# WujiangXu/AMID

Measured on AMD Instinct MI355X. Metric: train samples/sec, higher is better.
Workload: dtype f32; 1 GPU; cloth_sport_train75-shaped SASRec train step (BASELINE.json configs[1]); batch_per_gpu=256, global_batch=256, seq_len=50, emb_dim=128, hid_dim=32, neg=1, table_rows=894820, unique_rows_last_step=1921, input=HBM-resident batch pool, dropout=on (p=0.5), optimizer=Adam (dense-equivalent lazy rows), graph=True, steps_per_graph=1, parallelism=dp1

## Files before the change

amid_amd/csrc/sasrec_strip_px.hip:

```cpp
#include "common.h"
#include "rng.h"
#include "strip_gemm.h"
#include "strip_chain.h"
#include "seq_fwd.h"
#include "seq_bwd.h"
#include "seqn_parts.h"
#include "sort_phases.h"
#include "scorer_sum.h"
#include "strip_px.h"

namespace amid {

constexpr int PXB_WPS = 4, PXB_NS = 2, PXB_NW = PXB_WPS * PXB_NS, PXB_THREADS = 64 * PXB_NW;
constexpr int PXB_STAT_STRIP = 2 * 64 + 2 * 16, PXB_STAT = PXB_WPS * PXB_STAT_STRIP;
template <int D> constexpr size_t pxb_lds_floats(int chains = 1) {
    return (size_t)3 * (D * D / 2) + (size_t)PXB_WPS * XpStrip<D>::FLOATS + PXB_STAT + (size_t)chains * PXB_WPS * 2 * D;
}

struct PxbRow { unsigned off_own, phys; int local; bool ok; };
template <int D>
__device__ __forceinline__ PxbRow pxb_row(const StripGeom& sg, const StripTile& t, int si, int c0) {
    PxbRow r;
    int v = t.v0 + si * 16 + (lane_id() & 15);
    r.ok = v < t.nv;
    if (!r.ok) v = t.v0;
    if (sg.live != nullptr) {
        const int s = v / sg.T;
        r.local = sg.live[t.s0 + s] * sg.T + (v - s * sg.T);
    } else {
        r.local = v;
    }
    r.phys = (unsigned)t.g * (unsigned)sg.M + (unsigned)r.local;
    r.off_own = r.ok ? r.phys * (unsigned)(D * 4) + 16u * (unsigned)(lane_id() >> 4) + (unsigned)c0 * 64u : STRIP_OOB;
    return r;
}

template <class Add>
__device__ __forceinline__ void pxb_row_chain(float* __restrict__ stat, int si, int part, float& a, float& b, const Add& add) {
    typedef __attribute__((address_space(3))) float lf;
    float* ls = stat + si * PXB_STAT_STRIP;
    float* rs = ls + 2 * 64;
    const int lane = lane_id(), m = lane & 15;
    a = 0.f; b = 0.f;
    if (part == 0) { add(a, b); lds_st1(ls + lane, a); lds_st1(ls + 64 + lane, b); }
    lds_barrier();
    if (part != 0) {
        a = *(lf*)(ls + lane); b = *(lf*)(ls + 64 + lane);
        add(a, b);
        a = row_sum4(a); b = row_sum4(b);
        if (lane < 16) { lds_st1(rs + m, a); lds_st1(rs + 16 + m, b); }
    }
    lds_barrier();
    if (part == 0) { a = *(lf*)(rs + m); b = *(lf*)(rs + 16 + m); }
}

template <int D, int NCT>
__device__ __forceinline__ void pxb_ln_partials(float* __restrict__ scratch, int si, int c0, const PartRegs<NCT>& dgam, const PartRegs<NCT>& dbet) {
    const int lane = lane_id();
    float* mine = scratch + si * 2 * D;
#pragma unroll
    for (int c = 0; c < NCT; ++c) {
        f32x4 a, b;
#pragma unroll
        for (int r = 0; r < 4; ++r) { a[r] = col_sum16(dgam.v[c][r]); b[r] = col_sum16(dbet.v[c][r]); }
        if ((lane & 15) == 0) {
            lds_st4(mine + (c0 + c) * 16 + 4 * (lane >> 4), a);
            lds_st4(mine + D + (c0 + c) * 16 + 4 * (lane >> 4), b);
        }
    }
}
template <int D>
__device__ __forceinline__ void pxb_ln_partials_out(const float* __restrict__ scratch, float* __restrict__ part) {
    for (int e = threadIdx.x; e < 2 * D; e += PXB_THREADS)
        part[e] = (scratch[e] + scratch[2 * D + e]) + (scratch[4 * D + e] + scratch[6 * D + e]);
}

template <int D, int NCT>
__device__ __forceinline__ void pxb_ln_bwd(PartRegs<NCT>& DR, const PartRegs<NCT>& dbet, const PartRegs<NCT>& X, const PartRegs<NCT>& gam, bool have_stat,
                                           float mean, float& rstd, float eps, float* __restrict__ stat, int si, int part, PartRegs<NCT>& dgam,
                                           const f32x4 (*addend)[NCT] = nullptr, PartRegs<NCT>* uout = nullptr) {
    if (!have_stat) {
        float tot, qt, dummy;
        pxb_row_chain(stat, si, part, tot, dummy, [&](float& s, float&) {
#pragma unroll
            for (int c = 0; c < NCT; ++c) s += (X.v[c][0] + X.v[c][1]) + (X.v[c][2] + X.v[c][3]);
        });
        mean = tot * (1.0f / D);
        pxb_row_chain(stat, si, part, qt, dummy, [&](float& q, float&) {
#pragma unroll
            for (int c = 0; c < NCT; ++c)
#pragma unroll
                for (int r = 0; r < 4; ++r) { const float d = X.v[c][r] - mean; q = fmaf(d, d, q); }
        });
        rstd = 1.0f / sqrtf(qt * (1.0f / D) + eps);
    }
    float t1, t2;
    pxb_row_chain(stat, si, part, t1, t2, [&](float& s1, float& s2) {
#pragma unroll
        for (int c = 0; c < NCT; ++c) {
#pragma unroll
            for (int r = 0; r < 4; ++r) {
                const float dy = dbet.v[c][r];
                const float xh = (X.v[c][r] - mean) * rstd;
                float gy = gam.v[c][r] * dy;
                asm volatile("" : "+v"(gy));
                s1 += gy;
                s2 = fmaf(gy, xh, s2);
                float dg = dy * xh;
                asm volatile("" : "+v"(dg));
                dgam.v[c][r] = dg;
                DR.v[c][r] = gy;
            }
        }
    });
    const float c1 = t1 * (1.0f / D), c2 = t2 * (1.0f / D);
    {
#pragma clang fp contract(off)
#pragma unroll
        for (int c = 0; c < NCT; ++c)
#pragma unroll
            for (int r = 0; r < 4; ++r) {
                const float xh = (X.v[c][r] - mean) * rstd;
                const float u = __builtin_fmaf(-xh, c2, DR.v[c][r] - c1);
                if (uout != nullptr) uout->v[c][r] = u;
                DR.v[c][r] = addend != nullptr ? __builtin_fmaf(rstd, u, (*addend)[c][r]) : rstd * u;
            }
    }
}

template <int NCT>
__device__ __forceinline__ void xp_write_scaled(float* __restrict__ xps, int c0, const PartRegs<NCT>& u, float k) {
#pragma clang fp contract(off)
    const int lane = lane_id();
    auto split = [&](float ua, float ub) {
        WgSplit2 s;
        s.hi = wg_pack2(k * ua, k * ub);
        const float a1 = __builtin_fmaf(k, ua, -__uint_as_float(s.hi << 16)), b1 = __builtin_fmaf(k, ub, -__uint_as_float(s.hi & 0xffff0000u));
        s.mid = wg_pack2(a1, b1);
        const float a2 = a1 - __uint_as_float(s.mid << 16), b2 = b1 - __uint_as_float(s.mid & 0xffff0000u);
        s.lo = wg_pack2(a2, b2);
        return s;
    };
#pragma unroll
    for (int e = 0; e < NCT / 2; ++e) {
        const int st = c0 / 2 + e;
        const WgSplit2 p0 = split(u.v[2 * e][0], u.v[2 * e][1]), p1 = split(u.v[2 * e][2], u.v[2 * e][3]);
        const WgSplit2 p2 = split(u.v[2 * e + 1][0], u.v[2 * e + 1][1]), p3 = split(u.v[2 * e + 1][2], u.v[2 * e + 1][3]);
        lds_st4(xps + ((st * 3 + 0) * 64 + lane) * 4, __builtin_bit_cast(f32x4, amid_v4u{p0.hi, p1.hi, p2.hi, p3.hi}));
        lds_st4(xps + ((st * 3 + 1) * 64 + lane) * 4, __builtin_bit_cast(f32x4, amid_v4u{p0.mid, p1.mid, p2.mid, p3.mid}));
        lds_st4(xps + ((st * 3 + 2) * 64 + lane) * 4, __builtin_bit_cast(f32x4, amid_v4u{p0.lo, p1.lo, p2.lo, p3.lo}));
    }
}

template <int D, int NW> struct PxbRing : SeqRing3<D, NW> {
    using Base = SeqRing3<D, NW>;
    __device__ __forceinline__ explicit PxbRing(float* lds) : Base(lds) {}
    __device__ __forceinline__ void next() {
        w_ring_wait();
        __syncthreads();
        if (!this->hi_ready) this->plane(this->hslot(), this->cur);
    }
    __device__ __forceinline__ void mid_sync() {
        w_ring_wait();
        __syncthreads();
        this->plane(this->mslot(), this->nxt + (size_t)D * D);
        this->plane(this->lslot(), this->nxt + (size_t)2 * D * D);
        this->cur = this->nxt; this->hi_ready = false;
    }
};

template <int D, int NCT, class Ring>
__device__ __forceinline__ void pxb_mma_xp(f32x4 (&acc)[NCT], const float* __restrict__ xps, Ring& ring, int c0) {
    constexpr int KS = D / 32, NSTEP = KS * NCT, CT_BYTES = 16 * (D / 2) * 4, PLANE_BYTES = Ring::SLAB * 4;
    constexpr int PD1 = FRAG_AHEAD_2, PD2 = FRAG_AHEAD_1;
    static_assert(PD1 < NSTEP && PD2 < NSTEP && 2 * PD1 + 2 < 16, "read-ahead against the step count and the lgkmcnt field");
    const int lane = lane_id();
    const int i = lane & 15, g = lane >> 4;
    auto mma = [&](const f32x4& wf, const f32x4& a16, const f32x4& c) {
        return __builtin_amdgcn_mfma_f32_16x16x32_bf16(__builtin_bit_cast(seqn_bf16x8, wf), __builtin_bit_cast(seqn_bf16x8, a16), c, 0, 0, 0);
    };
    unsigned fo[KS];
#pragma unroll
    for (int s = 0; s < KS; ++s) fo[s] = (unsigned)((((c0 * 16 + i) * (D / 2)) + 4 * ((4 * s + g) ^ i)) * 4);
    const unsigned xa = lds_offset(xps) + (unsigned)lane * 16u;
    const unsigned mbase = lds_offset(ring.mslot());
    static_assert(CT_BYTES * (NCT - 1) + PLANE_BYTES < 65536, "the lo plane is reached through the offset field");
    const unsigned hbase = mbase + 2u * PLANE_BYTES;
    {
        f32x4 wm[PD1 + 1], wl[PD1 + 1], ah[KS], am[KS];
        static_for<KS>([&](auto S) {
            constexpr int s = decltype(S)::value;
            lds_frag_issue<(s * 3 + 0) * 1024>(ah[s], xa);
            lds_frag_issue<(s * 3 + 1) * 1024>(am[s], xa);
        });
        auto issue = [&](auto U) {
            constexpr int u = decltype(U)::value, c = u / KS, s = u % KS, k = u % (PD1 + 1);
            lds_frag_issue<c * CT_BYTES>(wm[k], mbase + fo[s]);
            lds_frag_issue<c * CT_BYTES + PLANE_BYTES>(wl[k], mbase + fo[s]);
        };
        static_for<PD1>(issue);
        static_for<NSTEP>([&](auto T) {
            constexpr int t = decltype(T)::value, c = t / KS, s = t % KS, k = t % (PD1 + 1);
            if constexpr (t + PD1 < NSTEP) issue(std::integral_constant<int, t + PD1>{});
            constexpr int last = t + PD1 < NSTEP ? t + PD1 : NSTEP - 1;
            asm volatile("s_waitcnt lgkmcnt(%4)" : "+v"(wm[k]), "+v"(wl[k]), "+v"(ah[s]), "+v"(am[s]) : "n"(2 * (last - t)));
            acc[c] = mma(wm[k], am[s], acc[c]); acc[c] = mma(wl[k], ah[s], acc[c]); acc[c] = mma(wm[k], ah[s], acc[c]);
        });
    }
    ring.mid_sync();
    {
        f32x4 wf[PD2 + 1], ah[KS], am[KS], al[KS];
        static_for<KS>([&](auto S) {
            constexpr int s = decltype(S)::value;
            lds_frag_issue<(s * 3 + 0) * 1024>(ah[s], xa);
            lds_frag_issue<(s * 3 + 1) * 1024>(am[s], xa);
            lds_frag_issue<(s * 3 + 2) * 1024>(al[s], xa);
        });
        auto issue = [&](auto U) {
            constexpr int u = decltype(U)::value, c = u / KS, s = u % KS;
            lds_frag_issue<c * CT_BYTES>(wf[u % (PD2 + 1)], hbase + fo[s]);
        };
        static_for<PD2>(issue);
        static_for<NSTEP>([&](auto T) {
            constexpr int t = decltype(T)::value, c = t / KS, s = t % KS, k = t % (PD2 + 1);
            if constexpr (t + PD2 < NSTEP) issue(std::integral_constant<int, t + PD2>{});
            constexpr int last = t + PD2 < NSTEP ? t + PD2 : NSTEP - 1;
            asm volatile("s_waitcnt lgkmcnt(%4)" : "+v"(wf[k]), "+v"(ah[s]), "+v"(am[s]), "+v"(al[s]) : "n"(last - t));
            acc[c] = mma(wf[k], al[s], acc[c]); acc[c] = mma(wf[k], am[s], acc[c]); acc[c] = mma(wf[k], ah[s], acc[c]);
        });
    }
}

template <int D, int NCT, bool ZERO = true, class Ring, class Stores>
__device__ __forceinline__ void pxb_product(f32x4 (&acc)[NCT], const float* __restrict__ xps, Ring& ring, const unsigned short* __restrict__ wn16, int c0,
                                            const Stores& stores) {
    if constexpr (ZERO) {
#pragma unroll
        for (int c = 0; c < NCT; ++c) acc[c] = f32x4{0.f, 0.f, 0.f, 0.f};
    }
    ring.begin(wn16);
#pragma unroll
    for (int ct = 0; ct < NCT; ++ct) { stores(ct, 1); stores(ct, 3); }
    pxb_mma_xp<D, NCT, Ring>(acc, xps, ring, c0);
}

template <int D, int NCT>
__device__ __forceinline__ void pxb_tm_load(unsigned (&bits)[NCT], const unsigned char* __restrict__ tmq, const StripGeom& sg, const PxbRow& row, int c0) {
    const GBuf gtm(tmq, sg.tm_bytes);
    const unsigned tbase = row.ok ? row.phys * (unsigned)(D / 4) + (unsigned)c0 * 4u : STRIP_OOB;
    const int sh = 8 * (lane_id() >> 4);
#pragma unroll
    for (int c = 0; c < NCT; ++c) bits[c] = (unsigned)__builtin_amdgcn_raw_buffer_load_b32(gtm.r, (int)(tbase + 4 * c), 0, 0) >> sh;
}
template <int NCT>
__device__ __forceinline__ void pxb_tm_apply(PartRegs<NCT>& x, const unsigned (&bits)[NCT]) {
#pragma unroll
    for (int c = 0; c < NCT; ++c) {
        x.v[c][0] = (bits[c] & 1u) ? 0.f : x.v[c][0];
        x.v[c][1] = (bits[c] & 2u) ? 0.f : x.v[c][1];
        x.v[c][2] = (bits[c] & 4u) ? 0.f : x.v[c][2];
        x.v[c][3] = (bits[c] & 8u) ? 0.f : x.v[c][3];
    }
}

template <int NCT> struct PxbFfnPre { PartRegs<NCT> Hs, gam; unsigned tm[NCT]; float mean, rstd; };
template <int D, int NCT>
__device__ __forceinline__ void pxb_ffn_prefetch(PxbFfnPre<NCT>& p, const StripFfnBwdArgs& a, const float* __restrict__ ln_stat, const StripGeom& sg,
                                                 const PxbRow& row, int g, int c0) {
    part_load<NCT>(p.Hs, GBuf(a.h, sg.act_bytes), row.off_own);
    if (a.tmq != nullptr) pxb_tm_load<D, NCT>(p.tm, a.tmq, sg, row, c0);
    part_cols<NCT>(p.gam, a.ln_w[g], c0);
    p.mean = 0.f; p.rstd = 0.f;
    if (ln_stat != nullptr && row.ok) { p.mean = ln_stat[(long long)row.phys * 4 + 2]; p.rstd = ln_stat[(long long)row.phys * 4 + 3]; }
}

template <int D, int NCT, class Ring>
__device__ __forceinline__ void pxb_ffn_bwd_chain(const StripFfnBwdArgs& a, const float* __restrict__ ln_stat, const StripGeom& sg, Ring& ring,
                                                  const PxbRow& row, int g, int si, int part, int c0, PartRegs<NCT>& DZ, PxbFfnPre<NCT>& pre,
                                                  float* __restrict__ xps, float* __restrict__ stat, float* __restrict__ lnsc,
                                                  const unsigned short* __restrict__ wnext) {
    const GBuf gp2(a.dpre2, sg.act_bytes), gp1(a.dpre1, sg.act_bytes), gdr(a.dr, sg.act_bytes), gdo(a.d_o, sg.act_bytes);
    PartRegs<NCT> P, Rs;
    PartRegs<NCT>& Hs = pre.Hs;
    PartRegs<NCT>& gam = pre.gam;
    float mean = pre.mean, rstd = pre.rstd;
    if (a.tmq != nullptr) pxb_tm_apply<NCT>(DZ, pre.tm);
    P = DZ;
    if (a.train) {
        const uint4 rr2 = rng_call(a.st->seed, (unsigned long long)row.local * D >> 7, site_id(g, a.layer, SITE_FFN2), (unsigned)a.st->step);
        part_dropout<NCT>(P, rr2, c0, a.spec, a.scale, (row.local * D) & 127);
    }
    xp_write<NCT>(xps, c0, P);
    f32x4 acc[NCT];
    {
        ring.next();
        part_load<NCT>(Rs, GBuf(a.r, sg.act_bytes), row.off_own);
        pxb_product<D, NCT>(acc, xps, ring, (const unsigned short*)a.w1T[g], c0, [&](int ct, int j) { part_spread<NCT>(gp2, row.off_own, P, ct, j, 1); });
#pragma unroll
        for (int c = 0; c < NCT; ++c)
#pragma unroll
            for (int r = 0; r < 4; ++r) P.v[c][r] = Hs.v[c][r] > 0.f ? acc[c][r] * a.scale : 0.f;
    }
    lds_barrier();
    xp_write<NCT>(xps, c0, P);
    PartRegs<NCT> DR, U, dgam, dbet;
    {
        ring.next();
        pxb_product<D, NCT>(acc, xps, ring, (const unsigned short*)a.woT[g], c0, [&](int ct, int j) { part_spread<NCT>(gp1, row.off_own, P, ct, j, 1); });
#pragma unroll
        for (int c = 0; c < NCT; ++c) dbet.v[c] = acc[c] + DZ.v[c];
        pxb_ln_bwd<D, NCT>(DR, dbet, Rs, gam, ln_stat != nullptr, mean, rstd, a.ln_eps, stat, si, part, dgam, nullptr, &U);
        pxb_ln_partials<D, NCT>(lnsc, si, c0, dgam, dbet);
    }
    xp_write_scaled<NCT>(xps, c0, U, rstd);
    {
        ring.next();
        pxb_product<D, NCT>(acc, xps, ring, wnext, c0, [&](int ct, int j) { part_spread<NCT>(gdr, row.off_own, DR, ct, j, 1); });
#pragma unroll
        for (int c = 0; c < NCT; ++c) P.v[c] = acc[c];
        part_store<NCT>(gdo, row.off_own, P);
    }
}

template <int D, int NCT, class Ring, class Hook>
__device__ __forceinline__ void pxb_qkv_bwd_chain(const StripQkvBwdArgs& a, const float* __restrict__ ln_stat, const StripGeom& sg, Ring& ring,
                                                  const PxbRow& row, int g, int si, int part, int c0, const PartRegs<NCT>& Dk, const PartRegs<NCT>& Dv,
                                                  PartRegs<NCT>& DX, float* __restrict__ xps, float* __restrict__ stat, float* __restrict__ lnsc,
                                                  const unsigned short* __restrict__ wnext, const Hook& before_last) {
    PartRegs<NCT> Dq, Drs, Xs, gam;
    f32x4 acc_kv[NCT], acc[NCT];
    const auto none = [](int, int) {};
    xp_write<NCT>(xps, c0, Dk);
    {
        ring.next();
        part_load<NCT>(Dq, GBuf(a.dq, sg.act_bytes), row.off_own);
        pxb_product<D, NCT>(acc_kv, xps, ring, (const unsigned short*)a.wvT[g], c0, none);
    }
    lds_barrier();
    xp_write<NCT>(xps, c0, Dv);
    float mean = 0.f, rstd = 0.f;
    {
        ring.next();
        part_load<NCT>(Drs, GBuf(a.dr, sg.act_bytes), row.off_own);
        part_load<NCT>(Xs, GBuf(a.x, sg.act_bytes), row.off_own);
        part_cols<NCT>(gam, a.ln_w[g], c0);
        if (ln_stat != nullptr && row.ok) { mean = ln_stat[(long long)row.phys * 4]; rstd = ln_stat[(long long)row.phys * 4 + 1]; }
        pxb_product<D, NCT, false>(acc_kv, xps, ring, (const unsigned short*)a.wqT[g], c0, none);
    }
    lds_barrier();
    xp_write<NCT>(xps, c0, Dq);
    PartRegs<NCT> dgam;
    {
        ring.next();
        before_last();
        pxb_product<D, NCT>(acc, xps, ring, wnext, c0, none);
#pragma unroll
        for (int c = 0; c < NCT; ++c) Drs.v[c] += acc[c];
        pxb_ln_bwd<D, NCT>(DX, Drs, Xs, gam, ln_stat != nullptr, mean, rstd, a.ln_eps, stat, si, part, dgam, &acc_kv);
    }
    pxb_ln_partials<D, NCT>(lnsc, si, c0, dgam, Drs);
}

struct PxbWave { int part, si, c0; };
template <int NCT> __device__ __forceinline__ PxbWave pxb_wave() {
    const int w = wave_id();
    return PxbWave{w / PXB_WPS, w % PXB_WPS, (w / PXB_WPS) * NCT};
}
template <int D> __device__ __forceinline__ float* pxb_xps(float* smem, int si) { return smem + 3 * SeqRing3<D, PXB_NW>::SLAB + si * XpStrip<D>::FLOATS; }
template <int D> __device__ __forceinline__ float* pxb_stat(float* smem) { return smem + 3 * SeqRing3<D, PXB_NW>::SLAB + PXB_WPS * XpStrip<D>::FLOATS; }
template <int D> __device__ __forceinline__ float* pxb_lnsc(float* smem, int which) { return pxb_stat<D>(smem) + PXB_STAT + which * PXB_WPS * 2 * D; }

template <int D, int RIDER>
__global__ __launch_bounds__(PXB_THREADS) void strip_ffn_bwd_px_kernel(const StripFfnBwdArgs a, const float* __restrict__ ln_stat, const StripGeom sg,
                                                                       const SortRider rd) {
    extern __shared__ __attribute__((aligned(16))) float smem[];
    constexpr int NCT = D / 16 / PXB_NS;
    int bid = blockIdx.x;
    if constexpr (RIDER != 0) {
        if (bid < rd.plan.nblk) { if (threadIdx.x < SORT_THREADS) sort_phase_ct<RIDER>(rd.plan, bid, smem); return; }
        bid -= rd.plan.nblk;
    }
    const PxbWave wv = pxb_wave<NCT>();
    const StripTile t = strip_tile(sg, bid);
    if (!t.live) { zero_slot<D>(a.ln_part, t.slot); return; }
    const int g = t.g;
    const PxbRow row = pxb_row<D>(sg, t, wv.si, wv.c0);
    PartRegs<NCT> DZ;
    PxbFfnPre<NCT> pre;
    part_load<NCT>(DZ, GBuf(a.dxo, sg.act_bytes), row.off_own);
    pxb_ffn_prefetch<D, NCT>(pre, a, ln_stat, sg, row, g, wv.c0);
    PxbRing<D, PXB_NW> ring(smem);
    ring.first((const unsigned short*)a.w2T[g]);
    float* const lnsc = pxb_lnsc<D>(smem, 0);
    pxb_ffn_bwd_chain<D, NCT>(a, ln_stat, sg, ring, row, g, wv.si, wv.part, wv.c0, DZ, pre, pxb_xps<D>(smem, wv.si), pxb_stat<D>(smem), lnsc,
                              (const unsigned short*)a.woT[g]);
    w_ring_wait();
    __syncthreads();
    pxb_ln_partials_out<D>(lnsc, a.ln_part + (long long)t.slot * 2 * D);
}

template <int D, bool FFN, int RIDER>
__global__ __launch_bounds__(PXB_THREADS) void strip_qkv_bwd_px_kernel(const StripQkvBwdArgs a, const StripFfnBwdArgs f, const float* __restrict__ ln_stat,
                                                                       const float* __restrict__ f_ln_stat, const ScorerSum ss, const StripGeom sg,
                                                                       const SortRider rd) {
    extern __shared__ __attribute__((aligned(16))) float smem[];
    constexpr int NCT = D / 16 / PXB_NS;
    int bid = blockIdx.x;
    if constexpr (RIDER != 0 && FFN) {
        if (ss.front) {
            if (bid < ss.nblk) { if (threadIdx.x < STRIP_THREADS) scorer_sum_block(ss, bid, (scorer_lds_f4*)smem); return; }
            bid -= ss.nblk;
        } else {
            const int first = (int)gridDim.x - ss.nblk;
            if (bid >= first) { if (threadIdx.x < STRIP_THREADS) scorer_sum_block(ss, bid - first, (scorer_lds_f4*)smem); return; }
        }
    }
    if constexpr (RIDER > 0) {
        if (bid < rd.plan.nblk) { if (threadIdx.x < SORT_THREADS) sort_phase_ct<RIDER>(rd.plan, bid, smem); return; }
        bid -= rd.plan.nblk;
    }
    const PxbWave wv = pxb_wave<NCT>();
    const StripTile t = strip_tile(sg, bid);
    if (!t.live) {
        zero_slot<D>(a.ln_part, t.slot);
        if constexpr (FFN) zero_slot<D>(f.ln_part, t.slot);
        return;
    }
    const int g = t.g;
    const PxbRow row = pxb_row<D>(sg, t, wv.si, wv.c0);
    PartRegs<NCT> Dk, Dv, DX;
    part_load<NCT>(Dk, GBuf(a.dk, sg.act_bytes), row.off_own);
    part_load<NCT>(Dv, GBuf(a.dv, sg.act_bytes), row.off_own);
    PxbRing<D, PXB_NW> ring(smem);
    ring.first((const unsigned short*)a.wkT[g]);
    float* const xps = pxb_xps<D>(smem, wv.si);
    float* const stat = pxb_stat<D>(smem);
    if constexpr (FFN) {
        PxbFfnPre<NCT> pre;
        pxb_qkv_bwd_chain<D, NCT>(a, ln_stat, sg, ring, row, g, wv.si, wv.part, wv.c0, Dk, Dv, DX, xps, stat, pxb_lnsc<D>(smem, 0),
                                  (const unsigned short*)f.w2T[g], [&]() { pxb_ffn_prefetch<D, NCT>(pre, f, f_ln_stat, sg, row, g, wv.c0); });
        pxb_ffn_bwd_chain<D, NCT>(f, f_ln_stat, sg, ring, row, g, wv.si, wv.part, wv.c0, DX, pre, xps, stat, pxb_lnsc<D>(smem, 1),
                                  (const unsigned short*)f.woT[g]);
    } else {
        const bool emb = a.emb_tmq != nullptr;
        unsigned etm[NCT];
        pxb_qkv_bwd_chain<D, NCT>(a, ln_stat, sg, ring, row, g, wv.si, wv.part, wv.c0, Dk, Dv, DX, xps, stat, pxb_lnsc<D>(smem, 0),
                                  (const unsigned short*)a.wkT[g], [&]() { if (emb) pxb_tm_load<D, NCT>(etm, a.emb_tmq, sg, row, wv.c0); });
        if (emb) {
            if (a.emb_train) {
                const uint4 rr = rng_call(a.emb_st->seed, (unsigned long long)row.local * D >> 7, site_id(g, 0, SITE_EMB), (unsigned)a.emb_st->step);
                part_dropout<NCT>(DX, rr, wv.c0, a.emb_spec, a.emb_scale, (row.local * D) & 127);
            }
            pxb_tm_apply<NCT>(DX, etm);
        }
        part_store<NCT>(GBuf(a.dx, sg.act_bytes), row.off_own, DX);
    }
    w_ring_wait();
    __syncthreads();
    pxb_ln_partials_out<D>(pxb_lnsc<D>(smem, 0), a.ln_part + (long long)t.slot * 2 * D);
    if constexpr (FFN) pxb_ln_partials_out<D>(pxb_lnsc<D>(smem, 1), f.ln_part + (long long)t.slot * 2 * D);
}

using namespace amid_strip_host;

static bool pxb_dropout_ok(int train, unsigned spec) { return !train || spec_bits(spec) == 1; }

int launch_ffn_bwd_px(const StripFfnBwdArgs& a, const float* ln_stat, const StripGeom& sg, const SortRider& rd, void* stream) {
    if (!pxb_dropout_ok(a.train, a.spec)) return AMID_ERR_UNSUPPORTED;
    if (rd.phase != 0 && rd.phase != 2) return AMID_ERR_UNSUPPORTED;
    constexpr size_t lds = pxb_lds_floats<128>() * sizeof(float);
    static_assert(lds >= sizeof(SortScatterLds<OS_BINS_MAX>), "the rider's scatter fits the head of the allocation");
    if (rd.phase != 0) return launch_lds<strip_ffn_bwd_px_kernel<128, 2>>(2 * sg.tpg + rd.plan.nblk, PXB_THREADS, lds, stream, a, ln_stat, sg, rd);
    return launch_lds<strip_ffn_bwd_px_kernel<128, 0>>(2 * sg.tpg, PXB_THREADS, lds, stream, a, ln_stat, sg, rd);
}

int launch_qkv_bwd_px(const StripQkvBwdArgs& a, const StripFfnBwdArgs& f, bool ffn, const float* ln_stat, const float* f_ln_stat, const ScorerSum& ss,
                      const StripGeom& sg, const SortRider& rd, void* stream) {
    if (!pxb_dropout_ok(a.emb_train, a.emb_spec) || (ffn && !pxb_dropout_ok(f.train, f.spec))) return AMID_ERR_UNSUPPORTED;
    if (rd.phase != 0 && rd.phase != (ffn ? 3 : 4)) return AMID_ERR_UNSUPPORTED;
    if (ss.nblk > 0 && !ffn) return AMID_ERR_UNSUPPORTED;
    constexpr size_t lds1 = pxb_lds_floats<128>(1) * sizeof(float), lds2 = pxb_lds_floats<128>(2) * sizeof(float);
    static_assert(lds2 <= 160 * 1024, "the fused launch's second LayerNorm scratch fits the CU's LDS");
    static_assert(lds1 >= sizeof(SortScatterLds<OS_BINS_MAX>) && lds1 >= 8 * 33 * 16, "a rider's scratch fits the head of the allocation");
    const int tiles = 2 * sg.tpg, sortb = rider_blocks_host(rd);
    if (ffn) {
        if (rd.phase) return launch_lds<strip_qkv_bwd_px_kernel<128, true, 3>>(tiles + sortb + ss.nblk, PXB_THREADS, lds2, stream, a, f, ln_stat, f_ln_stat, ss, sg, rd);
        return launch_lds<strip_qkv_bwd_px_kernel<128, true, -1>>(tiles + ss.nblk, PXB_THREADS, lds2, stream, a, f, ln_stat, f_ln_stat, ss, sg, rd);
    }
    if (rd.phase) return launch_lds<strip_qkv_bwd_px_kernel<128, false, 4>>(tiles + sortb, PXB_THREADS, lds1, stream, a, f, ln_stat, f_ln_stat, ss, sg, rd);
    return launch_lds<strip_qkv_bwd_px_kernel<128, false, 0>>(tiles, PXB_THREADS, lds1, stream, a, f, ln_stat, f_ln_stat, ss, sg, rd);
}

}

using namespace amid;
using namespace amid_strip_host;

extern "C" int amid_sas_strip_ffn_bwd_px_f32(const float* dxo, const unsigned char* tmq, const float* h, const float* r, const float* const* ln_w,
                                             const float* const* w1T, const float* const* w2T, const float* const* woT, float ln_eps, int B, int T,
                                             int D, const int* live, int layer, const void* step_state, int train, float p_drop, float* dpre2,
                                             float* dpre1, float* dr, float* d_o, float* ln_part, const float* ln_stat, const void* sort_plan,
                                             int sort_phase, void* stream) {
    AMID_FFN_BWD_CALL(c);
    AMID_CHECK_ARG(c.dxo && c.operands());
    if (D != 128) return AMID_ERR_UNSUPPORTED;
    if (train && p_drop > 0.f && spec_bits(drop_spec(p_drop)) != 1) return AMID_ERR_UNSUPPORTED;
    StripGeom sg;
    if (int e = make_strip_geom(B, T, D, live, &sg)) return e;
    StripFfnBwdArgs a;
    fill_ffn_bwd(a, c);
    SortRider rd;
    rd.phase = 0;
    if (sort_plan != nullptr) {
        if (sort_phase != 2) return AMID_ERR_UNSUPPORTED;
        rd.plan = *(const SortPlan*)sort_plan;
        rd.phase = sort_phase;
    }
    return launch_ffn_bwd_px(a, ln_stat, sg, rd, stream);
}
#undef AMID_FFN_BWD_CALL
```

amid_amd/csrc/seqn_parts.h:

```cpp
#pragma once
#include "common.h"
#include "rng.h"
#include "strip_gemm.h"
#include "bf16_pieces.h"
#include <type_traits>
#include "seq_fwd.h"

namespace amid {

typedef __attribute__((address_space(3))) float lds_f;
typedef float lds_v4 __attribute__((ext_vector_type(4)));
__device__ __forceinline__ float4 lds_ld4(const float* p) {
    const lds_v4 t = *(const __attribute__((address_space(3))) lds_v4*)(p);
    return make_float4(t.x, t.y, t.z, t.w);
}
__device__ __forceinline__ void lds_st4(float* p, f32x4 v) { *(__attribute__((address_space(3))) lds_v4*)(p) = lds_v4{v[0], v[1], v[2], v[3]}; }
__device__ __forceinline__ void lds_st1(float* p, float v) { *(__attribute__((address_space(3))) float*)(p) = v; }

template <int D, int NW> struct WDmaN {
    static constexpr int CPR = D / 4;
    static constexpr int PER_WAVE = D * CPR / 64 / NW;
    static constexpr unsigned STRIDE2 = 2u * (NW * 64 / CPR) * D * 4;
    unsigned off[2];
    int w;
// ... 311 lines not shown
    }
    if constexpr (std::is_same<Ring, SeqRing16x3<D, Ring::NWAVES>>::value) {
        ring.begin(wn16);
        late();
        part_mma16x6<D, NCT>(acc, A, ring, c0);
#pragma unroll
        for (int ct = 0; ct < NCT; ++ct) { stores(ct, 1); stores(ct, 3); }
    } else if constexpr (BF) {
        ring.fetch_all(wn16);
        late();
        part_mma16<D, NCT>(acc, A, buf, c0);
#pragma unroll
        for (int ct = 0; ct < NCT; ++ct) { stores(ct, 1); stores(ct, 3); }
    } else {
        part_mma<D, NCT>(acc, A, buf, c0, [&](int ct, int j) {
            ring.fetch(wn32, ct, j);
            stores(ct, j);
            if (ct == D / 16 / 2 && j == 0) late();
        });
    }
}

template <int D, int NW> struct SeqRing3 {
    static constexpr int NWAVES = NW;
    static constexpr int CPR = D / 8;
    static constexpr int PIECES = D * CPR / 64, PER_WAVE = PIECES / NW;
    static constexpr int SLAB = D * D / 2;
    float* buf; unsigned off0; int w;
    const unsigned short* cur; const unsigned short* nxt;
    bool hi_ready, rest_ready, rest_late, hold_next;
    bool one;
    __device__ __forceinline__ explicit SeqRing3(float* lds)
        : buf(lds), cur(nullptr), nxt(nullptr), hi_ready(false), rest_ready(false), rest_late(false), hold_next(false), one(false) {
        w = wave_id();
        const int p = w * 64 + lane_id();
        const int n = p / CPR, pos = p % CPR;
        off0 = (unsigned)(n * D * 2 + ((pos ^ (n & 15)) * 16));
    }
    __device__ __forceinline__ float* mslot() const { return buf; }
    __device__ __forceinline__ float* lslot() const { return buf + SLAB; }
    __device__ __forceinline__ float* hslot() const { return buf + 2 * SLAB; }
    __device__ __forceinline__ float* images() const { return buf; }
    __device__ __forceinline__ void piece(float* __restrict__ dst, const unsigned short* __restrict__ W, int k0) const {
        const unsigned voff = off0 + (unsigned)k0 * (unsigned)(NW * 64 / CPR) * (unsigned)(D * 2);
        const unsigned lds = __builtin_amdgcn_readfirstlane(
            lds_offset(dst + (k0 * NW + w) * 256));
        unsigned keep;
        asm volatile("s_mov_b32 %0, m0\n\ts_mov_b32 m0, %3\n\ts_nop 2\n\tglobal_load_lds_dwordx4 %1, %2\n\ts_mov_b32 m0, %0"
                     : "=&s"(keep) : "v"(voff), "s"(W), "s"(lds) : "memory");
    }
    __device__ __forceinline__ void plane(float* __restrict__ dst, const unsigned short* __restrict__ Wp) const {
#pragma unroll
        for (int k0 = 0; k0 < PER_WAVE; ++k0) piece(dst, Wp, k0);
    }
    __device__ __forceinline__ void first(const unsigned short* __restrict__ W0) {
        cur = W0; hi_ready = true; rest_ready = true;
        plane(hslot(), W0);
        if (!one) { plane(mslot(), W0 + (size_t)D * D); plane(lslot(), W0 + (size_t)2 * D * D); }
    }
    __device__ __forceinline__ void next() {
        w_ring_wait();
        __syncthreads();
        if (!hi_ready) plane(hslot(), cur);
        rest_late = !hi_ready;
        if (!rest_ready && !one) { plane(mslot(), cur + (size_t)D * D); plane(lslot(), cur + (size_t)2 * D * D); }
        hold_next = false;
    }
    __device__ __forceinline__ void begin(const unsigned short* __restrict__ Wnext) { nxt = Wnext; }
    __device__ __forceinline__ void pre_pass1() {
        if (rest_late) { w_ring_wait(); __syncthreads(); }
    }
    __device__ __forceinline__ void mid_sync() {
#ifndef AMID_XNOWAIT
        w_ring_wait();
#endif
        __syncthreads();
        plane(hslot(), nxt);
        cur = nxt; hi_ready = true; rest_ready = false;
    }
};

template <int D> struct XpStrip { static constexpr int FLOATS = (D / 32) * 3 * 64 * 4; };
template <int NCT>
__device__ __forceinline__ void xp_write(float* __restrict__ xps, int c0, const PartRegs<NCT>& x) {
    static_assert(NCT % 2 == 0, "a wave owns whole k-steps (pairs of column tiles)");
    const int lane = lane_id();
#pragma unroll
    for (int e = 0; e < NCT / 2; ++e) {
        const int s = c0 / 2 + e;
        const WgSplit2 p0 = wg_split3(x.v[2 * e][0], x.v[2 * e][1]), p1 = wg_split3(x.v[2 * e][2], x.v[2 * e][3]);
        const WgSplit2 p2 = wg_split3(x.v[2 * e + 1][0], x.v[2 * e + 1][1]), p3 = wg_split3(x.v[2 * e + 1][2], x.v[2 * e + 1][3]);
        lds_st4(xps + ((s * 3 + 0) * 64 + lane) * 4, __builtin_bit_cast(f32x4, amid_v4u{p0.hi, p1.hi, p2.hi, p3.hi}));
        lds_st4(xps + ((s * 3 + 1) * 64 + lane) * 4, __builtin_bit_cast(f32x4, amid_v4u{p0.mid, p1.mid, p2.mid, p3.mid}));
        lds_st4(xps + ((s * 3 + 2) * 64 + lane) * 4, __builtin_bit_cast(f32x4, amid_v4u{p0.lo, p1.lo, p2.lo, p3.lo}));
    }
}
__device__ __forceinline__ amid_v4u xp_frag(const float* __restrict__ xps, int s, int p) {
    const float4 t = lds_ld4(xps + ((s * 3 + p) * 64 + lane_id()) * 4);
    return __builtin_bit_cast(amid_v4u, t);
}
template <int D>
__device__ __forceinline__ void xp_row(StripRegs<D>& full, const float* __restrict__ xps) {
#pragma unroll
    for (int s = 0; s < D / 32; ++s) {
        const amid_v4u h = xp_frag(xps, s, 0), m = xp_frag(xps, s, 1), l = xp_frag(xps, s, 2);
#pragma unroll
        for (int j = 0; j < 4; ++j) {
            const float lo = (__uint_as_float(h[j] << 16) + __uint_as_float(m[j] << 16)) + __uint_as_float(l[j] << 16);
            const float hi = (__uint_as_float(h[j] & 0xffff0000u) + __uint_as_float(m[j] & 0xffff0000u)) + __uint_as_float(l[j] & 0xffff0000u);
            full.v[2 * s + (j >> 1)][2 * (j & 1)] = lo;
            full.v[2 * s + (j >> 1)][2 * (j & 1) + 1] = hi;
        }
    }
}

template <int D, int NCT, class Ring, bool ONE = false>
__device__ __forceinline__ void part_mma_xp(f32x4 (&acc)[NCT], const float* __restrict__ xps, Ring& ring, int c0) {
    constexpr int KS = D / 32, NSTEP = KS * NCT, CT_BYTES = 16 * (D / 2) * 4, PLANE_BYTES = Ring::SLAB * 4;
    constexpr int PD1 = FRAG_AHEAD_2, PD2 = FRAG_AHEAD_1;
    static_assert(PD1 < NSTEP && PD2 < NSTEP && 2 * PD1 + 2 < 16, "read-ahead against the step count and the lgkmcnt field");
    const int lane = lane_id();
    const int i = lane & 15, g = lane >> 4;
    auto lds_addr = [](const float* p) { return lds_offset(p); };
    auto mma = [&](const f32x4& wf, const f32x4& a16, const f32x4& c) {
        return __builtin_amdgcn_mfma_f32_16x16x32_bf16(__builtin_bit_cast(seqn_bf16x8, wf), __builtin_bit_cast(seqn_bf16x8, a16), c, 0, 0, 0);
    };
    unsigned fo[KS];
#pragma unroll
    for (int s = 0; s < KS; ++s) fo[s] = (unsigned)((((c0 * 16 + i) * (D / 2)) + 4 * ((4 * s + g) ^ i)) * 4);
    const unsigned xa = lds_addr(xps) + (unsigned)lane * 16u;
    const unsigned mbase = lds_addr(ring.mslot());
    static_assert(CT_BYTES * (NCT - 1) + PLANE_BYTES < 65536, "the lo plane is reached through the offset field");
    const unsigned hbase = mbase + 2u * PLANE_BYTES;
    ring.pre_pass1();
    {
        f32x4 wf[PD2 + 1], ah[KS], am[KS], al[KS];
        static_for<KS>([&](auto S) {
            constexpr int s = decltype(S)::value;
            lds_frag_issue<(s * 3 + 0) * 1024>(ah[s], xa);
            lds_frag_issue<(s * 3 + 1) * 1024>(am[s], xa);
            lds_frag_issue<(s * 3 + 2) * 1024>(al[s], xa);
        });
        auto issue = [&](auto U) {
            constexpr int u = decltype(U)::value, c = u / KS, s = u % KS;
            lds_frag_issue<c * CT_BYTES>(wf[u % (PD2 + 1)], hbase + fo[s]);
        };
        static_for<PD2>(issue);
        static_for<NSTEP>([&](auto T) {
            constexpr int t = decltype(T)::value, c = t / KS, s = t % KS, k = t % (PD2 + 1);
            if constexpr (t + PD2 < NSTEP) issue(std::integral_constant<int, t + PD2>{});
            constexpr int last = t + PD2 < NSTEP ? t + PD2 : NSTEP - 1;
            asm volatile("s_waitcnt lgkmcnt(%4)" : "+v"(wf[k]), "+v"(ah[s]), "+v"(am[s]), "+v"(al[s]) : "n"(last - t));
            if constexpr (!ONE) { acc[c] = mma(wf[k], al[s], acc[c]); acc[c] = mma(wf[k], am[s], acc[c]); }
            acc[c] = mma(wf[k], ah[s], acc[c]);
        });
    }
    ring.mid_sync();
    if constexpr (!ONE) {
        f32x4 wm[PD1 + 1], wl[PD1 + 1], ah[KS], am[KS];
        static_for<KS>([&](auto S) {
            constexpr int s = decltype(S)::value;
            lds_frag_issue<(s * 3 + 0) * 1024>(ah[s], xa);
            lds_frag_issue<(s * 3 + 1) * 1024>(am[s], xa);
        });
        auto issue = [&](auto U) {
            constexpr int u = decltype(U)::value, c = u / KS, s = u % KS, k = u % (PD1 + 1);
            lds_frag_issue<c * CT_BYTES>(wm[k], mbase + fo[s]);
            lds_frag_issue<c * CT_BYTES + PLANE_BYTES>(wl[k], mbase + fo[s]);
        };
        static_for<PD1>(issue);
        static_for<NSTEP>([&](auto T) {
            constexpr int t = decltype(T)::value, c = t / KS, s = t % KS, k = t % (PD1 + 1);
            if constexpr (t + PD1 < NSTEP) issue(std::integral_constant<int, t + PD1>{});
            constexpr int last = t + PD1 < NSTEP ? t + PD1 : NSTEP - 1;
            asm volatile("s_waitcnt lgkmcnt(%4)" : "+v"(wm[k]), "+v"(wl[k]), "+v"(ah[s]), "+v"(am[s]) : "n"(2 * (last - t)));
            acc[c] = mma(wl[k], ah[s], acc[c]); acc[c] = mma(wm[k], am[s], acc[c]); acc[c] = mma(wm[k], ah[s], acc[c]);
        });
    }
// ... 31 lines not shown
```

Baseline: 903,500 samples/s.

## Overlap weight-plane DMA and next-operand LDS writes with MFMA steps in strip backward

```diff
diff --git a/amid_amd/csrc/sasrec_strip_px.hip b/amid_amd/csrc/sasrec_strip_px.hip
--- a/amid_amd/csrc/sasrec_strip_px.hip
+++ b/amid_amd/csrc/sasrec_strip_px.hip
@@ -10,6 +10,13 @@
 #include "strip_px.h"
 
 namespace amid {
+
+#ifdef AMID_STRIP_STAMPS
+static __device__ unsigned long long amid_pxb_stamp_buf[8 * 64];
+#define PXB_STAMP(i) do { if (blockIdx.x == 0 && lane_id() == 0) amid_pxb_stamp_buf[wave_id() * 64 + (i)] = __builtin_amdgcn_s_memrealtime(); } while (0)
+#else
+#define PXB_STAMP(i) do { } while (0)
+#endif
 
 constexpr int PXB_WPS = 4, PXB_NS = 2, PXB_NW = PXB_WPS * PXB_NS, PXB_THREADS = 64 * PXB_NW;
 constexpr int PXB_STAT_STRIP = 2 * 64 + 2 * 16, PXB_STAT = PXB_WPS * PXB_STAT_STRIP;
@@ -154,23 +161,72 @@
 
 template <int D, int NW> struct PxbRing : SeqRing3<D, NW> {
     using Base = SeqRing3<D, NW>;
-    __device__ __forceinline__ explicit PxbRing(float* lds) : Base(lds) {}
+    bool hi_flying;
+    __device__ __forceinline__ explicit PxbRing(float* lds) : Base(lds), hi_flying(false) {}
+    template <int N> static __device__ __forceinline__ void wait_but() { asm volatile("s_waitcnt vmcnt(%0)" ::"n"(N) : "memory"); }
+    __device__ __forceinline__ void request_hi() {
+#ifndef AMID_PXB_PARENT_SCHEDULE
+        if (!this->hi_ready) { this->plane(this->hslot(), this->cur); this->hi_ready = true; hi_flying = true; }
+#endif
+    }
     __device__ __forceinline__ void next() {
+#ifdef AMID_PXB_PARENT_SCHEDULE
         w_ring_wait();
         __syncthreads();
+#else
+        if (hi_flying) wait_but<Base::PER_WAVE>(); else w_ring_wait();
+        lds_barrier();
+#endif
         if (!this->hi_ready) this->plane(this->hslot(), this->cur);
     }
-    __device__ __forceinline__ void mid_sync() {
+    template <class Landed>
+    __device__ __forceinline__ void mid_sync(const Landed& landed) {
         w_ring_wait();
         __syncthreads();
+        landed();
+#ifdef AMID_PXB_PARENT_SCHEDULE
         this->plane(this->mslot(), this->nxt + (size_t)D * D);
         this->plane(this->lslot(), this->nxt + (size_t)2 * D * D);
-        this->cur = this->nxt; this->hi_ready = false;
+#endif
+        this->cur = this->nxt; this->hi_ready = false; hi_flying = false;
+    }
+    static constexpr int ML_PIECES = 2 * Base::PER_WAVE;
+    __device__ __forceinline__ void ml_piece(int j) {
+#ifndef AMID_PXB_PARENT_SCHEDULE
+        if (j < Base::PER_WAVE) this->piece(this->mslot(), this->cur + (size_t)D * D, j);
+        else this->piece(this->lslot(), this->cur + (size_t)2 * D * D, j - Base::PER_WAVE);
+#endif
     }
 };
 
-template <int D, int NCT, class Ring>
-__device__ __forceinline__ void pxb_mma_xp(f32x4 (&acc)[NCT], const float* __restrict__ xps, Ring& ring, int c0) {
+template <int NCT> __device__ __forceinline__ void pxb_pin(PartRegs<NCT>& x) {
+#pragma unroll
+    for (int c = 0; c < NCT; ++c) asm volatile("" : "+v"(x.v[c]));
+}
+struct PxbNoUnder {
+    static constexpr bool on = false;
+    __device__ __forceinline__ void landed() const {}
+    __device__ __forceinline__ void kstep(int) const {}
+};
+template <class F> struct PxbLanded {
+    static constexpr bool on = false;
+    const F& f;
+    __device__ __forceinline__ void landed() const { f(); }
+    __device__ __forceinline__ void kstep(int) const {}
+};
+template <class F> __device__ __forceinline__ PxbLanded<F> pxb_landed(const F& f) { return PxbLanded<F>{f}; }
+template <int NCT, bool EARLY> struct PxbFromMemory {
+    static constexpr bool on = EARLY;
+    float* xps; int c0; PartRegs<NCT>& x;
+    __device__ __forceinline__ void landed() const { pxb_pin<NCT>(x); }
+    __device__ __forceinline__ void kstep(int e) const {
+        asm volatile("" : "+v"(x.v[2 * e]), "+v"(x.v[2 * e + 1]));
+        xp_write_kstep<NCT>(xps, c0, x, e);
+    }
+};
+
+template <int D, int NCT, int SB, class Ring, class Under>
+__device__ __forceinline__ void pxb_mma_xp(f32x4 (&acc)[NCT], const float* __restrict__ xps, Ring& ring, int c0, const Under& under) {
     constexpr int KS = D / 32, NSTEP = KS * NCT, CT_BYTES = 16 * (D / 2) * 4, PLANE_BYTES = Ring::SLAB * 4;
     constexpr int PD1 = FRAG_AHEAD_2, PD2 = FRAG_AHEAD_1;
     static_assert(PD1 < NSTEP && PD2 < NSTEP && 2 * PD1 + 2 < 16, "read-ahead against the step count and the lgkmcnt field");
@@ -186,8 +242,10 @@
     const unsigned mbase = lds_offset(ring.mslot());
     static_assert(CT_BYTES * (NCT - 1) + PLANE_BYTES < 65536, "the lo plane is reached through the offset field");
     const unsigned hbase = mbase + 2u * PLANE_BYTES;
-    {
-        f32x4 wm[PD1 + 1], wl[PD1 + 1], ah[KS], am[KS];
+    f32x4 ah[KS], am[KS], al[KS];
+    if constexpr (SB >= 0) PXB_STAMP(SB);
+    {
+        f32x4 wm[PD1 + 1], wl[PD1 + 1];
         static_for<KS>([&](auto S) {
             constexpr int s = decltype(S)::value;
             lds_frag_issue<(s * 3 + 0) * 1024>(ah[s], xa);
@@ -207,15 +265,24 @@
             acc[c] = mma(wm[k], am[s], acc[c]); acc[c] = mma(wl[k], ah[s], acc[c]); acc[c] = mma(wm[k], ah[s], acc[c]);
         });
     }
-    ring.mid_sync();
-    {
-        f32x4 wf[PD2 + 1], ah[KS], am[KS], al[KS];
-        static_for<KS>([&](auto S) {
-            constexpr int s = decltype(S)::value;
-            lds_frag_issue<(s * 3 + 0) * 1024>(ah[s], xa);
-            lds_frag_issue<(s * 3 + 1) * 1024>(am[s], xa);
-            lds_frag_issue<(s * 3 + 2) * 1024>(al[s], xa);
-        });
+    if constexpr (SB >= 0) PXB_STAMP(SB + 1);
+    if constexpr (Under::on) {
+        static_for<KS>([&](auto S) { constexpr int s = decltype(S)::value; lds_frag_issue<(s * 3 + 2) * 1024>(al[s], xa); });
+        static_assert(KS == 4, "the wait names every lo fragment");
+        asm volatile("s_waitcnt lgkmcnt(0)" : "+v"(al[0]), "+v"(al[1]), "+v"(al[2]), "+v"(al[3]));
+    }
+    ring.mid_sync([&]() { under.landed(); });
+    if constexpr (SB >= 0) PXB_STAMP(SB + 2);
+    {
+        f32x4 wf[PD2 + 1];
+        if constexpr (!Under::on) {
+            static_for<KS>([&](auto S) {
+                constexpr int s = decltype(S)::value;
+                lds_frag_issue<(s * 3 + 0) * 1024>(ah[s], xa);
+                lds_frag_issue<(s * 3 + 1) * 1024>(am[s], xa);
+                lds_frag_issue<(s * 3 + 2) * 1024>(al[s], xa);
+            });
+        }
         auto issue = [&](auto U) {
             constexpr int u = decltype(U)::value, c = u / KS, s = u % KS;
             lds_frag_issue<c * CT_BYTES>(wf[u % (PD2 + 1)], hbase + fo[s]);
@@ -227,13 +294,18 @@
             constexpr int last = t + PD2 < NSTEP ? t + PD2 : NSTEP - 1;
             asm volatile("s_waitcnt lgkmcnt(%4)" : "+v"(wf[k]), "+v"(ah[s]), "+v"(am[s]), "+v"(al[s]) : "n"(last - t));
             acc[c] = mma(wf[k], al[s], acc[c]); acc[c] = mma(wf[k], am[s], acc[c]); acc[c] = mma(wf[k], ah[s], acc[c]);
+            constexpr int ML_EVERY = NSTEP / Ring::ML_PIECES;
+            if constexpr (t % ML_EVERY == 0 && t / ML_EVERY < Ring::ML_PIECES) ring.ml_piece(t / ML_EVERY);
+            constexpr int EVERY = NSTEP / (NCT / 2);
+            if constexpr (Under::on && t % EVERY == 1) under.kstep(t / EVERY);
         });
     }
-}
-
-template <int D, int NCT, bool ZERO = true, class Ring, class Stores>
+    if constexpr (SB >= 0) PXB_STAMP(SB + 3);
+}
+
+template <int D, int NCT, int SB, bool ZERO = true, class Ring, class Stores, class Under = PxbNoUnder>
 __device__ __forceinline__ void pxb_product(f32x4 (&acc)[NCT], const float* __restrict__ xps, Ring& ring, const unsigned short* __restrict__ wn16, int c0,
-                                            const Stores& stores) {
+                                            const Stores& stores, const Under& under = Under()) {
     if constexpr (ZERO) {
 #pragma unroll
         for (int c = 0; c < NCT; ++c) acc[c] = f32x4{0.f, 0.f, 0.f, 0.f};
@@ -241,7 +313,7 @@
     ring.begin(wn16);
 #pragma unroll
     for (int ct = 0; ct < NCT; ++ct) { stores(ct, 1); stores(ct, 3); }
-    pxb_mma_xp<D, NCT, Ring>(acc, xps, ring, c0);
+    pxb_mma_xp<D, NCT, SB>(acc, xps, ring, c0, under);
 }
 
 template <int D, int NCT>
@@ -272,6 +344,14 @@
     part_cols<NCT>(p.gam, a.ln_w[g], c0);
     p.mean = 0.f; p.rstd = 0.f;
     if (ln_stat != nullptr && row.ok) { p.mean = ln_stat[(long long)row.phys * 4 + 2]; p.rstd = ln_stat[(long long)row.phys * 4 + 3]; }
+}
+
+template <int NCT> __device__ __forceinline__ void pxb_ffn_pin(PxbFfnPre<NCT>& p, bool tm) {
+    pxb_pin<NCT>(p.Hs); pxb_pin<NCT>(p.gam);
+    if (tm) {
+#pragma unroll
+        for (int c = 0; c < NCT; ++c) asm volatile("" : "+v"(p.tm[c]));
+    }
 }
 
 template <int D, int NCT, class Ring>
@@ -291,74 +371,101 @@
         part_dropout<NCT>(P, rr2, c0, a.spec, a.scale, (row.local * D) & 127);
     }
     xp_write<NCT>(xps, c0, P);
+    PXB_STAMP(25);
     f32x4 acc[NCT];
     {
         ring.next();
+        PXB_STAMP(26);
         part_load<NCT>(Rs, GBuf(a.r, sg.act_bytes), row.off_own);
-        pxb_product<D, NCT>(acc, xps, ring, (const unsigned short*)a.w1T[g], c0, [&](int ct, int j) { part_spread<NCT>(gp2, row.off_own, P, ct, j, 1); });
+        pxb_product<D, NCT, 27>(acc, xps, ring, (const unsigned short*)a.w1T[g], c0, [&](int ct, int j) { part_spread<NCT>(gp2, row.off_own, P, ct, j, 1); });
 #pragma unroll
         for (int c = 0; c < NCT; ++c)
 #pragma unroll
             for (int r = 0; r < 4; ++r) P.v[c][r] = Hs.v[c][r] > 0.f ? acc[c][r] * a.scale : 0.f;
     }
     lds_barrier();
+    ring.request_hi();
     xp_write<NCT>(xps, c0, P);
+    PXB_STAMP(31);
     PartRegs<NCT> DR, U, dgam, dbet;
     {
         ring.next();
-        pxb_product<D, NCT>(acc, xps, ring, (const unsigned short*)a.woT[g], c0, [&](int ct, int j) { part_spread<NCT>(gp1, row.off_own, P, ct, j, 1); });
+        PXB_STAMP(32);
+        pxb_product<D, NCT, 33>(acc, xps, ring, (const unsigned short*)a.woT[g], c0, [&](int ct, int j) { part_spread<NCT>(gp1, row.off_own, P, ct, j, 1); },
+                                    pxb_landed([&]() { pxb_pin<NCT>(Rs); }));
 #pragma unroll
         for (int c = 0; c < NCT; ++c) dbet.v[c] = acc[c] + DZ.v[c];
         pxb_ln_bwd<D, NCT>(DR, dbet, Rs, gam, ln_stat != nullptr, mean, rstd, a.ln_eps, stat, si, part, dgam, nullptr, &U);
+        ring.request_hi();
         pxb_ln_partials<D, NCT>(lnsc, si, c0, dgam, dbet);
     }
+    PXB_STAMP(37);
     xp_write_scaled<NCT>(xps, c0, U, rstd);
+    PXB_STAMP(38);
     {
         ring.next();
-        pxb_product<D, NCT>(acc, xps, ring, wnext, c0, [&](int ct, int j) { part_spread<NCT>(gdr, row.off_own, DR, ct, j, 1); });
+        PXB_STAMP(39);
+        pxb_product<D, NCT, 40>(acc, xps, ring, wnext, c0, [&](int ct, int j) { part_spread<NCT>(gdr, row.off_own, DR, ct, j, 1); });
 #pragma unroll
         for (int c = 0; c < NCT; ++c) P.v[c] = acc[c];
         part_store<NCT>(gdo, row.off_own, P);
     }
-}
-
-template <int D, int NCT, class Ring, class Hook>
+    PXB_STAMP(44);
+}
+
+#ifdef AMID_PXB_PARENT_SCHEDULE
+constexpr bool PXB_EARLY_XP = false;
+#else
+constexpr bool PXB_EARLY_XP = true;
+#endif
+template <int D, int NCT, class Ring, class Hook, class After>
 __device__ __forceinline__ void pxb_qkv_bwd_chain(const StripQkvBwdArgs& a, const float* __restrict__ ln_stat, const StripGeom& sg, Ring& ring,
-                                                  const PxbRow& row, int g, int si, int part, int c0, const PartRegs<NCT>& Dk, const PartRegs<NCT>& Dv,
+                                                  const PxbRow& row, int g, int si, int part, int c0, const PartRegs<NCT>& Dk, PartRegs<NCT>& Dv,
                                                   PartRegs<NCT>& DX, float* __restrict__ xps, float* __restrict__ stat, float* __restrict__ lnsc,
-                                                  const unsigned short* __restrict__ wnext, const Hook& before_last) {
+                                                  const unsigned short* __restrict__ wnext, const Hook& before_last, const After& after_ln) {
     PartRegs<NCT> Dq, Drs, Xs, gam;
     f32x4 acc_kv[NCT], acc[NCT];
     const auto none = [](int, int) {};
+    const auto under = [&](PartRegs<NCT>& next) { return PxbFromMemory<NCT, PXB_EARLY_XP>{xps, c0, next}; };
+    const auto late = [&](const PartRegs<NCT>& next) {
+        if constexpr (!PXB_EARLY_XP) { lds_barrier(); ring.request_hi(); xp_write<NCT>(xps, c0, next); }
+    };
     xp_write<NCT>(xps, c0, Dk);
+    PXB_STAMP(2);
     {
         ring.next();
+        PXB_STAMP(3);
         part_load<NCT>(Dq, GBuf(a.dq, sg.act_bytes), row.off_own);
-        pxb_product<D, NCT>(acc_kv, xps, ring, (const unsigned short*)a.wvT[g], c0, none);
-    }
-    lds_barrier();
-    xp_write<NCT>(xps, c0, Dv);
+        pxb_product<D, NCT, 4>(acc_kv, xps, ring, (const unsigned short*)a.wvT[g], c0, none, under(Dv));
+    }
+    late(Dv);
+    PXB_STAMP(8);
     float mean = 0.f, rstd = 0.f;
     {
         ring.next();
+        PXB_STAMP(9);
         part_load<NCT>(Drs, GBuf(a.dr, sg.act_bytes), row.off_own);
         part_load<NCT>(Xs, GBuf(a.x, sg.act_bytes), row.off_own);
         part_cols<NCT>(gam, a.ln_w[g], c0);
         if (ln_stat != nullptr && row.ok) { mean = ln_stat[(long long)row.phys * 4]; rstd = ln_stat[(long long)row.phys * 4 + 1]; }
-        pxb_product<D, NCT, false>(acc_kv, xps, ring, (const unsigned short*)a.wqT[g], c0, none);
-    }
-    lds_barrier();
-    xp_write<NCT>(xps, c0, Dq);
+        pxb_product<D, NCT, 10, false>(acc_kv, xps, ring, (const unsigned short*)a.wqT[g], c0, none, under(Dq));
+    }
+    late(Dq);
+    PXB_STAMP(14);
     PartRegs<NCT> dgam;
     {
         ring.next();
+        PXB_STAMP(15);
         before_last();
-        pxb_product<D, NCT>(acc, xps, ring, wnext, c0, none);
+        pxb_product<D, NCT, 16>(acc, xps, ring, wnext, c0, none, pxb_landed([&]() { pxb_pin<NCT>(Drs); pxb_pin<NCT>(Xs); pxb_pin<NCT>(gam); }));
 #pragma unroll
         for (int c = 0; c < NCT; ++c) Drs.v[c] += acc[c];
         pxb_ln_bwd<D, NCT>(DX, Drs, Xs, gam, ln_stat != nullptr, mean, rstd, a.ln_eps, stat, si, part, dgam, &acc_kv);
-    }
+        after_ln();
+    }
+    PXB_STAMP(20);
     pxb_ln_partials<D, NCT>(lnsc, si, c0, dgam, Drs);
+    PXB_STAMP(21);
 }
 
 struct PxbWave { int part, si, c0; };
@@ -387,16 +494,20 @@
     const PxbRow row = pxb_row<D>(sg, t, wv.si, wv.c0);
     PartRegs<NCT> DZ;
     PxbFfnPre<NCT> pre;
+    PXB_STAMP(0);
     part_load<NCT>(DZ, GBuf(a.dxo, sg.act_bytes), row.off_own);
     pxb_ffn_prefetch<D, NCT>(pre, a, ln_stat, sg, row, g, wv.c0);
     PxbRing<D, PXB_NW> ring(smem);
     ring.first((const unsigned short*)a.w2T[g]);
+    PXB_STAMP(1);
     float* const lnsc = pxb_lnsc<D>(smem, 0);
     pxb_ffn_bwd_chain<D, NCT>(a, ln_stat, sg, ring, row, g, wv.si, wv.part, wv.c0, DZ, pre, pxb_xps<D>(smem, wv.si), pxb_stat<D>(smem), lnsc,
                               (const unsigned short*)a.woT[g]);
     w_ring_wait();
     __syncthreads();
+    PXB_STAMP(61);
     pxb_ln_partials_out<D>(lnsc, a.ln_part + (long long)t.slot * 2 * D);
+    PXB_STAMP(62);
 }
 
 template <int D, bool FFN, int RIDER>
@@ -429,23 +540,26 @@
     const int g = t.g;
     const PxbRow row = pxb_row<D>(sg, t, wv.si, wv.c0);
     PartRegs<NCT> Dk, Dv, DX;
+    PXB_STAMP(0);
     part_load<NCT>(Dk, GBuf(a.dk, sg.act_bytes), row.off_own);
     part_load<NCT>(Dv, GBuf(a.dv, sg.act_bytes), row.off_own);
     PxbRing<D, PXB_NW> ring(smem);
     ring.first((const unsigned short*)a.wkT[g]);
+    PXB_STAMP(1);
     float* const xps = pxb_xps<D>(smem, wv.si);
     float* const stat = pxb_stat<D>(smem);
     if constexpr (FFN) {
         PxbFfnPre<NCT> pre;
         pxb_qkv_bwd_chain<D, NCT>(a, ln_stat, sg, ring, row, g, wv.si, wv.part, wv.c0, Dk, Dv, DX, xps, stat, pxb_lnsc<D>(smem, 0),
-                                  (const unsigned short*)f.w2T[g], [&]() { pxb_ffn_prefetch<D, NCT>(pre, f, f_ln_stat, sg, row, g, wv.c0); });
+                                        (const unsigned short*)f.w2T[g], [&]() { pxb_ffn_prefetch<D, NCT>(pre, f, f_ln_stat, sg, row, g, wv.c0); },
+                                  [&]() { pxb_ffn_pin<NCT>(pre, f.tmq != nullptr); ring.request_hi(); });
         pxb_ffn_bwd_chain<D, NCT>(f, f_ln_stat, sg, ring, row, g, wv.si, wv.part, wv.c0, DX, pre, xps, stat, pxb_lnsc<D>(smem, 1),
                                   (const unsigned short*)f.woT[g]);
     } else {
         const bool emb = a.emb_tmq != nullptr;
         unsigned etm[NCT];
         pxb_qkv_bwd_chain<D, NCT>(a, ln_stat, sg, ring, row, g, wv.si, wv.part, wv.c0, Dk, Dv, DX, xps, stat, pxb_lnsc<D>(smem, 0),
-                                  (const unsigned short*)a.wkT[g], [&]() { if (emb) pxb_tm_load<D, NCT>(etm, a.emb_tmq, sg, row, wv.c0); });
+                                         (const unsigned short*)a.wkT[g], [&]() { if (emb) pxb_tm_load<D, NCT>(etm, a.emb_tmq, sg, row, wv.c0); }, []() {});
         if (emb) {
             if (a.emb_train) {
                 const uint4 rr = rng_call(a.emb_st->seed, (unsigned long long)row.local * D >> 7, site_id(g, 0, SITE_EMB), (unsigned)a.emb_st->step);
@@ -455,10 +569,13 @@
         }
         part_store<NCT>(GBuf(a.dx, sg.act_bytes), row.off_own, DX);
     }
+    PXB_STAMP(60);
     w_ring_wait();
     __syncthreads();
+    PXB_STAMP(61);
     pxb_ln_partials_out<D>(pxb_lnsc<D>(smem, 0), a.ln_part + (long long)t.slot * 2 * D);
     if constexpr (FFN) pxb_ln_partials_out<D>(pxb_lnsc<D>(smem, 1), f.ln_part + (long long)t.slot * 2 * D);
+    PXB_STAMP(62);
 }
 
 using namespace amid_strip_host;
@@ -495,6 +612,12 @@
 
 using namespace amid;
 using namespace amid_strip_host;
+
+#ifdef AMID_STRIP_STAMPS
+extern "C" int amid_pxb_stamps_read(unsigned long long* host) {
+    return (int)hipMemcpyFromSymbol(host, HIP_SYMBOL(amid::amid_pxb_stamp_buf), sizeof(unsigned long long) * 8 * 64);
+}
+#endif
 
 extern "C" int amid_sas_strip_ffn_bwd_px_f32(const float* dxo, const unsigned char* tmq, const float* h, const float* r, const float* const* ln_w,
                                              const float* const* w1T, const float* const* w2T, const float* const* woT, float ln_eps, int B, int T,
diff --git a/amid_amd/csrc/seqn_parts.h b/amid_amd/csrc/seqn_parts.h
--- a/amid_amd/csrc/seqn_parts.h
+++ b/amid_amd/csrc/seqn_parts.h
@@ -417,18 +417,19 @@
 
 template <int D> struct XpStrip { static constexpr int FLOATS = (D / 32) * 3 * 64 * 4; };
 template <int NCT>
+__device__ __forceinline__ void xp_write_kstep(float* __restrict__ xps, int c0, const PartRegs<NCT>& x, int e) {
+    const int lane = lane_id(), s = c0 / 2 + e;
+    const WgSplit2 p0 = wg_split3(x.v[2 * e][0], x.v[2 * e][1]), p1 = wg_split3(x.v[2 * e][2], x.v[2 * e][3]);
+    const WgSplit2 p2 = wg_split3(x.v[2 * e + 1][0], x.v[2 * e + 1][1]), p3 = wg_split3(x.v[2 * e + 1][2], x.v[2 * e + 1][3]);
+    lds_st4(xps + ((s * 3 + 0) * 64 + lane) * 4, __builtin_bit_cast(f32x4, amid_v4u{p0.hi, p1.hi, p2.hi, p3.hi}));
+    lds_st4(xps + ((s * 3 + 1) * 64 + lane) * 4, __builtin_bit_cast(f32x4, amid_v4u{p0.mid, p1.mid, p2.mid, p3.mid}));
+    lds_st4(xps + ((s * 3 + 2) * 64 + lane) * 4, __builtin_bit_cast(f32x4, amid_v4u{p0.lo, p1.lo, p2.lo, p3.lo}));
+}
+template <int NCT>
 __device__ __forceinline__ void xp_write(float* __restrict__ xps, int c0, const PartRegs<NCT>& x) {
     static_assert(NCT % 2 == 0, "a wave owns whole k-steps (pairs of column tiles)");
-    const int lane = lane_id();
-#pragma unroll
-    for (int e = 0; e < NCT / 2; ++e) {
-        const int s = c0 / 2 + e;
-        const WgSplit2 p0 = wg_split3(x.v[2 * e][0], x.v[2 * e][1]), p1 = wg_split3(x.v[2 * e][2], x.v[2 * e][3]);
-        const WgSplit2 p2 = wg_split3(x.v[2 * e + 1][0], x.v[2 * e + 1][1]), p3 = wg_split3(x.v[2 * e + 1][2], x.v[2 * e + 1][3]);
-        lds_st4(xps + ((s * 3 + 0) * 64 + lane) * 4, __builtin_bit_cast(f32x4, amid_v4u{p0.hi, p1.hi, p2.hi, p3.hi}));
-        lds_st4(xps + ((s * 3 + 1) * 64 + lane) * 4, __builtin_bit_cast(f32x4, amid_v4u{p0.mid, p1.mid, p2.mid, p3.mid}));
-        lds_st4(xps + ((s * 3 + 2) * 64 + lane) * 4, __builtin_bit_cast(f32x4, amid_v4u{p0.lo, p1.lo, p2.lo, p3.lo}));
-    }
+#pragma unroll
+    for (int e = 0; e < NCT / 2; ++e) xp_write_kstep<NCT>(xps, c0, x, e);
 }
 __device__ __forceinline__ amid_v4u xp_frag(const float* __restrict__ xps, int s, int p) {
     const float4 t = lds_ld4(xps + ((s * 3 + p) * 64 + lane_id()) * 4);
```

Result: no change. 909,300 samples/s, median of 6 (+0.6%).
